# SobeyMIL/MVOC

Measured on AMD Instinct MI355X. Metric: UNet3D denoising steps/sec, 16x512^2 frames, inversion+compose, higher is better.
Workload: dtype f16

## Files before the change

### mvoc_amd/build.py

```python
import hashlib
import os
import subprocess
import sys

HERE = os.path.dirname(os.path.abspath(__file__))
CSRC = os.path.join(HERE, "csrc")
LIB = os.path.join(HERE, "libmvoc_hip.so")
SOURCES = ["runtime.hip", "gemm.hip", "gemm8.hip", "attention.hip", "tfused.hip", "xslin.hip", "norm.hip", "pnp.hip", "pnp_variants2.hip", "pnp_warp.hip", "stem.hip", "comm.hip",
           "pnp_bilinear.hip", "collage.hip"]
HIPCC = os.environ.get("HIPCC", "/opt/rocm/bin/hipcc")
LAB = os.environ.get("MVOC_BUILD_LAB") == "1"
if LAB:
    LIB = os.path.join(HERE, "libmvoc_hip_lab.so")
VARIANT = os.environ.get("MVOC_BUILD_VARIANT", "")
VARIANT_DEFS = os.environ.get("MVOC_BUILD_DEFS", "").split()
if VARIANT:
    LIB = os.path.join(HERE, f"libmvoc_hip_{VARIANT}.so")
FLAGS = ["--offload-arch=gfx950", "-O3", "-std=c++17", "-fPIC", "-fno-gpu-rdc", "-Wall", "-Wno-unused-function",
         "-ffp-contract=on", "-Rpass-analysis=kernel-resource-usage"]
EXTRA_FLAGS = {"attention.hip": ["-mllvm", "-amdgpu-mfma-vgpr-form"], "gemm.hip": ["-mllvm", "-amdgpu-mfma-vgpr-form"],
               "gemm8.hip": ["-mllvm", "-amdgpu-mfma-vgpr-form", "-falign-loops=64"], "tfused.hip": ["-mllvm", "-amdgpu-mfma-vgpr-form"],
               "xslin.hip": ["-mllvm", "-amdgpu-mfma-vgpr-form"]}


def _digest():
    h = hashlib.sha256()
    for f in sorted(x for x in os.listdir(CSRC) if x.endswith((".hip", ".h"))) + ["../../include/mvoc_hip.h"]:
        with open(os.path.join(CSRC, f), "rb") as fh:
            h.update(fh.read())
    h.update((" ".join(FLAGS + VARIANT_DEFS) + repr(sorted(EXTRA_FLAGS.items()))).encode())
    return h.hexdigest()


def build(force=False, verbose=True):
    stamp = LIB + ".stamp"
    dig = _digest()
    if not force and os.path.exists(LIB) and os.path.exists(stamp) and open(stamp).read() == dig:
        return LIB
    objs = []
    procs = []
    shared = b"".join(open(os.path.join(CSRC, f), "rb").read() for f in sorted(os.listdir(CSRC)) if f.endswith(".h"))
    shared += open(os.path.join(HERE, "..", "include", "mvoc_hip.h"), "rb").read()
    for src in SOURCES:
        obj = os.path.join(CSRC, src.replace(".hip", f".{VARIANT}.o" if VARIANT else (".lab.o" if LAB else ".o")))
        objs.append(obj)
        cmd = [HIPCC, *FLAGS, *(["-DMVOC_PP_LAB"] if LAB else []), *VARIANT_DEFS, *EXTRA_FLAGS.get(src, []), "-c", os.path.join(CSRC, src), "-o", obj]
        od = hashlib.sha256(open(os.path.join(CSRC, src), "rb").read() + shared + " ".join(cmd).encode()).hexdigest()
        ostamp = obj + ".stamp"
        if not force and os.path.exists(obj) and os.path.exists(ostamp) and open(ostamp).read() == od:
            continue
        if verbose:
            print(" ".join(cmd), flush=True)
        procs.append((src, subprocess.Popen(cmd, stdout=subprocess.PIPE, stderr=subprocess.STDOUT, text=True), ostamp, od))
    failed = False
    for src, p, ostamp, od in procs:
        out, _ = p.communicate()
        remarks = "\n".join(l for l in out.splitlines() if "-Rpass-analysis=kernel-resource-usage" in l)
        out = "\n".join(l for l in out.splitlines() if "-Rpass-analysis=kernel-resource-usage" not in l)
        with open(ostamp.replace(".stamp", ".res.txt"), "w") as fh:
            fh.write(remarks + "\n")
        if out.strip() and verbose:
            print(out)
        if p.returncode != 0:
            failed = True
            print(f"hipcc failed on {src}:\n{out}", file=sys.stderr)
        else:
            with open(ostamp, "w") as fh:
                fh.write(od)
    if failed:
        raise RuntimeError("libmvoc_hip.so: compilation failed")
    cmd = [HIPCC, "--offload-arch=gfx950", "-shared", "-fPIC", "-o", LIB, *objs, "-ldl"]
    if verbose:
        print(" ".join(cmd), flush=True)
    subprocess.run(cmd, check=True)
    with open(stamp, "w") as fh:
        fh.write(dig)
    return LIB


if __name__ == "__main__":
    build(force="--force" in sys.argv)
```

### mvoc_amd/csrc/gemm.hip

```cpp
#include <stdlib.h>

#include "gemm_args.h"

namespace {

constexpr int BK = 32;
constexpr int ROWB = 80;

struct RowInfo {
  int m;
  int y0, x0;
  int img;
};

template <int WN, int WM, int TN, int TM>
__device__ __forceinline__ void gemm_epilogue(const GemmArgs& p, f32x16 (&acc)[TN][TM], int n0, int m0, int wn, int wm,
                                              int r, int h, const float* lnstat = nullptr) {
#pragma unroll
  for (int j = 0; j < TM; ++j) {
    const int m = m0 + (wm * TM + j) * 32 + r;
    if (m >= p.M) continue;
    const half_t* ra = p.rowadd ? p.rowadd + (size_t)(m / p.rowadd_div) * p.ld_rowadd : nullptr;
    const half_t* rs = p.resid ? p.resid + (size_t)m * p.ldr : nullptr;
    half_t* orow = p.out + (size_t)m * p.ldo;
// ... 703 lines not shown
  for (int i = 0; i < 8; ++i) {
    const int m = blockIdx.x * 256 + rg + 32 * i;
    f32x4 a = {0.f, 0.f, 0.f, 0.f};
    for (int s = 0; s < p.split_k; ++s) a += *reinterpret_cast<const f32x4*>(p.ws + ((size_t)s * p.M + m) * p.N + n);
    float v[4];
#pragma unroll
    for (int e = 0; e < 4; ++e) v[e] = r16(a[e] + bs[e]);
    if (p.rowadd) {
      const half4_t ra = *reinterpret_cast<const half4_t*>(p.rowadd + (size_t)(m / p.rowadd_div) * p.ld_rowadd + n);
#pragma unroll
      for (int e = 0; e < 4; ++e) v[e] = r16(v[e] + (float)ra[e]);
    }
    if (p.resid) {
      const half4_t rs = *reinterpret_cast<const half4_t*>(p.resid + (size_t)m * p.ldr + n);
#pragma unroll
      for (int e = 0; e < 4; ++e) v[e] = r16(v[e] + (float)rs[e]);
    }
    const half4_t o4 = {(half_t)v[0], (half_t)v[1], (half_t)v[2], (half_t)v[3]};
    *reinterpret_cast<half4_t*>(p.out + (size_t)m * p.ldo + n) = o4;
#pragma unroll
    for (int e = 0; e < 4; ++e) {
      const float f = (float)o4[e];
      sx[e] += f;
      sq[e] += f * f;
    }
  }
#pragma unroll
  for (int e = 0; e < 4; ++e) {
    ls[rg][4 * cq + e] = sx[e];
    lq[rg][4 * cq + e] = sq[e];
  }
  __syncthreads();
  if (tid < 64) {
    const int c = tid & 31;
    const float(*src)[33] = tid < 32 ? ls : lq;
    float acc = 0.f;
#pragma unroll
    for (int g = 0; g < 32; ++g) acc += src[g][c];
    p.stats[((size_t)blockIdx.x * p.n_store + blockIdx.y * 32 + c) * 2 + (tid >> 5)] = acc;
  }
}

template <int WN, int WM, int TN, int TM, int NST = 2, int PF = 0, int BKK = 64, int PLAIN = 0>
int launch_glds(const GemmArgs& a0, hipStream_t s) {
  GemmArgs a = a0;
  constexpr int BN = WN * TN * 32, BM = WM * TM * 32;
  a.n_tiles = (a.N + BN - 1) / BN;
  a.m_tiles = (a.M + BM - 1) / BM;
  const long nblk = (long)a.n_tiles * a.m_tiles;
  if (nblk <= 0 || nblk > 0x7fffffffL) {
    mvoc_set_error("gemm: grid of %ld blocks", nblk);
    return -2;
  }
  constexpr bool HOT = (WN == 2 && WM == 2 && TN == 2 && TM == 2) || (WN == 1 && WM == 4 && TM == 1 && (TN == 2 || TN == 5));
  if (HOT && a.epi_lds && !a.ln_s && a.act == MVOC_ACT_NONE && a.split_k == 1) {
    if constexpr (HOT) {
      hipLaunchKernelGGL((gemm_glds_kernel<WN, WM, TN, TM, NST, PF, BKK, PLAIN, 1>), dim3((unsigned)nblk), dim3(WN * WM * 64), 0, s, a);
      return mvoc_check_launch("gemm_glds_kernel (plain epilogue)");
    }
  }
  hipLaunchKernelGGL((gemm_glds_kernel<WN, WM, TN, TM, NST, PF, BKK, PLAIN>), dim3((unsigned)(nblk * a.split_k)), dim3(WN * WM * 64), 0, s, a);
  if (a.split_k > 1) {
    if (a.stats) {
      hipLaunchKernelGGL(splitk_reduce_sums_kernel, dim3((unsigned)(a.M / 256), (unsigned)(a.N / 32)), dim3(256), 0, s, a);
    } else {
      const long nthr = (long)a.M * (a.N / 4);
      hipLaunchKernelGGL(splitk_reduce_kernel, dim3((unsigned)((nthr + 255) / 256)), dim3(256), 0, s, a);
    }
  }
  return mvoc_check_launch("gemm_glds_kernel");
}

}

extern "C" size_t mvoc_gemm_workspace_bytes(int64_t m, int64_t n, int64_t k) {
  if (m <= 0 || n <= 0 || k < 2048 || m > 8192) return 0;
  return (size_t)8 * (size_t)m * (size_t)n * sizeof(float);
}

namespace {
thread_local int g_sums_written = 0;
thread_local int g_rowmom_bx = 0;
const bool g_trace = getenv("MVOC_GEMM_TRACE") != nullptr;
}
extern "C" int mvoc_gemm_chan_sums_written(void) { return g_sums_written; }
extern "C" int mvoc_gemm_row_moments_written(void) { return g_rowmom_bx; }

namespace {
bool sums_reduce_ok(const mvoc_gemm_desc* d) {
  return d->ldo % 4 == 0 && ((uintptr_t)d->out & 7) == 0 && (!d->resid || (d->ldr % 4 == 0 && ((uintptr_t)d->resid & 7) == 0)) &&
         (!d->rowadd || (d->ld_rowadd % 4 == 0 && ((uintptr_t)d->rowadd & 7) == 0));
}

int gemm_dispatch(const mvoc_gemm_desc* d, void* stream) {
  g_sums_written = 0;
  g_rowmom_bx = 0;
  MVOC_REQUIRE(d && d->a && d->w && d->out, -1, "gemm: null operand");
  MVOC_REQUIRE(d->m > 0 && d->n > 0 && d->k > 0, -1, "gemm: empty problem m=%ld n=%ld k=%ld", (long)d->m, (long)d->n,
               (long)d->k);
  MVOC_REQUIRE(d->m < (1LL << 31) && d->n < (1 << 24) && d->k < (1 << 24), -2, "gemm: problem too large");
  MVOC_REQUIRE(d->n % 32 == 0 && d->k % BK == 0, -2, "gemm: n (%ld) must be a multiple of 32 and k (%ld) of %d",
               (long)d->n, (long)d->k, BK);
  MVOC_REQUIRE(d->cin > 0 && d->cin % 8 == 0 && d->c1 % 8 == 0 && d->c1 <= d->cin, -2,
               "gemm: cin (%d) and c1 (%d) must be multiples of 8", d->cin, d->c1);
  MVOC_REQUIRE(d->a2 || d->c1 == d->cin, -1, "gemm: c1 < cin needs a second source");
  MVOC_REQUIRE(d->a_mode >= 0 && d->a_mode <= 2, -1, "gemm: bad a_mode %d", d->a_mode);
  MVOC_REQUIRE(d->ldo % 4 == 0 && (d->resid == nullptr || d->ldr % 4 == 0), -2, "gemm: ldo/ldr must be multiples of 4");
  GemmArgs a;
  memset(&a, 0, sizeof(a));
  a.a = (const half_t*)d->a; a.a2 = (const half_t*)d->a2; a.w = (const half_t*)d->w; a.out = (half_t*)d->out;
  a.bias = (const half_t*)d->bias; a.rowadd = (const half_t*)d->rowadd; a.resid = (const half_t*)d->resid;
  a.M = (int)d->m; a.N = (int)d->n; a.K = (int)d->k;
  a.n_store = d->n_store > 0 ? d->n_store : (int)d->n;
  a.ldo = d->ldo; a.ldr = d->ldr; a.ld_rowadd = d->ld_rowadd; a.rowadd_div = d->rowadd_div > 0 ? d->rowadd_div : 1;
  a.a_mode = d->a_mode; a.lda = d->lda; a.lda2 = d->lda2; a.c1 = d->c1; a.cin = d->cin;
  a.nimg = d->nimg; a.hout = d->hout; a.wout = d->wout; a.hsrc = d->hsrc; a.wsrc = d->wsrc;
  a.stride = d->stride > 0 ? d->stride : 1; a.upsample = d->upsample;
  a.pad = d->pad_mode == 1 ? 0 : 1;
  a.hup = d->upsample ? d->hup : d->hsrc; a.wup = d->upsample ? d->wup : d->wsrc;
  a.ups_sh = d->upsample ? (float)d->hsrc / (float)d->hup : 1.f;
  a.ups_sw = d->upsample ? (float)d->wsrc / (float)d->wup : 1.f;
  a.frames = d->frames; a.hw = d->hw; a.act = d->act;
  a.split_k = 1; a.k_per_split = (int)d->k; a.ws = nullptr;
  a.ln_s = (const float*)d->ln_rowsum; a.ln_c = (const float*)d->ln_bias; a.ln_eps = d->ln_eps;
  a.ln_stats = (const float*)d->ln_stats;
  {
    const int ns = d->act == MVOC_ACT_GEGLU ? (int)d->n / 2 : (d->n_store > 0 ? d->n_store : (int)d->n);
    a.epi_lds = d->ldo % 8 == 0 && ns % 8 == 0 && ((uintptr_t)d->out & 15) == 0 &&
                (d->resid == nullptr || (d->ldr % 8 == 0 && ((uintptr_t)d->resid & 15) == 0));
  }
  if (d->a_mode == MVOC_A_CONV3X3) {
    MVOC_REQUIRE(d->nimg > 0 && d->hout > 0 && d->wout > 0 && d->hsrc > 0 && d->wsrc > 0, -1, "gemm: conv dims");
    MVOC_REQUIRE((int64_t)d->nimg * d->hout * d->wout == d->m, -1, "gemm: conv m != nimg*hout*wout");
    MVOC_REQUIRE(d->upsample == 2 || d->k >= 9 * (int64_t)d->cin, -1, "gemm: conv k < 9*cin");
    MVOC_REQUIRE(d->pad_mode == 0 || (d->pad_mode == 1 && !d->upsample), -1, "gemm: pad_mode %d", d->pad_mode);
    if (d->upsample == 2) {
      const int64_t spr = (int64_t)d->nimg * d->hsrc * d->wsrc;
      MVOC_REQUIRE(d->hup == 2 * d->hsrc && d->wup == 2 * d->wsrc && d->hout == d->hup && d->wout == d->wup && d->stride <= 1 &&
                       d->k == 4 * (int64_t)d->cin && spr % 256 == 0 && d->a2 == nullptr && d->resid == nullptr && d->rowadd == nullptr &&
                       d->act == MVOC_ACT_NONE && !d->ln_rowsum && d->split_k <= 1 && d->m >= 1024 && (d->tile == 0 || d->tile == 81),
                   -2, "gemm: upsample == 2 (sub-pixel) needs an exact 2x upsample, k == 4 cin, one source, nimg * hsrc * wsrc %% 256 == 0, "
                       "the plain epilogue, no split-K and m >= 1024");
      a.subpx = 1;
      a.sp_rows = (int)spr;
      a.hout = d->hsrc; a.wout = d->wsrc;
      a.hup = d->hsrc; a.wup = d->wsrc;
    }
  } else if (d->a_mode == MVOC_A_TEMPORAL3) {
    MVOC_REQUIRE(d->frames > 0 && d->hw > 0 && d->m % ((int64_t)d->frames * d->hw) == 0, -1, "gemm: temporal dims");
    MVOC_REQUIRE(d->k == 3 * (int64_t)d->cin, -1, "gemm: temporal k != 3*cin");
  } else {
    MVOC_REQUIRE(d->k == d->cin, -1, "gemm: plain mode needs cin == k");
  }
  if (d->act == MVOC_ACT_GEGLU) {
    MVOC_REQUIRE(d->n % 64 == 0, -2, "gemm: GEGLU needs n %% 64 == 0");
    a.n_store = (int)d->n / 2;
  }
  hipStream_t s = (hipStream_t)stream;
  const double flops = 2.0 * (double)d->m * (double)d->n * (double)d->k;
  MvocProfScope prof(MVOC_FAM_GEMM, s, flops);
  const bool glds_ok = d->k % 64 == 0 && d->cin % 64 == 0 && d->c1 % 64 == 0 &&
                       (d->a_mode != MVOC_A_CONV3X3 || d->k == (d->upsample == 2 ? 4 : 9) * (int64_t)d->cin);
  if (d->ln_rowsum) {
    MVOC_REQUIRE(d->ln_bias && d->ln_stats && glds_ok && d->a_mode == MVOC_A_PLAIN && d->a2 == nullptr && d->split_k <= 1 &&
                     (d->tile == 0 || d->tile >= 11),
                 -2, "gemm: LayerNorm folding needs the rows' statistics (ln_stats, mvoc_row_stats_f16) and the plain single-source "
                     "direct-to-LDS path (k %% 64 == 0), no split-K");
  }
  int tile = d->tile;
  int model_sk = 0, g8_sk = 0;
  const int conc = d->concurrency < 1 ? 1 : (d->concurrency > 8 ? 8 : d->concurrency);
  const int64_t rows_a = d->a_mode == MVOC_A_CONV3X3 ? (int64_t)d->nimg * d->hsrc * d->wsrc : d->m;
  const int64_t lim = (int64_t)1 << 31;
  const bool g8_ok = glds_ok && a.epi_lds && (a.n_store % 8 == 0) &&
                     rows_a * d->lda * 2 < lim && (d->a2 == nullptr || rows_a * d->lda2 * 2 < lim) &&
                     (int64_t)d->n * d->k * 2 < lim &&
                     (int64_t)d->m * d->ldo * 2 < lim && (!d->resid || (int64_t)d->m * d->ldr * 2 < lim) &&
                     ((uintptr_t)d->bias & 15) == 0 && ((uintptr_t)d->ln_rowsum & 15) == 0 && ((uintptr_t)d->ln_bias & 15) == 0 &&
                     (!d->rowadd || (((uintptr_t)d->rowadd & 15) == 0 && d->ld_rowadd % 8 == 0 && a.rowadd_div >= 64)) &&
                     (!d->upsample || (d->act == MVOC_ACT_NONE && !d->ln_rowsum));
  if (d->k_order) {
    MVOC_REQUIRE(d->k_order == 1 && d->a_mode != MVOC_A_PLAIN && !d->upsample && g8_ok && d->m >= 1024 && (tile == 0 || tile == 82) &&
                     d->k == (d->a_mode == MVOC_A_CONV3X3 ? 9 : 3) * (int64_t)d->cin && d->n % 320 == 0 && d->act == MVOC_ACT_NONE &&
                     !d->ln_rowsum && d->split_k <= 1 &&
                     (d->a_mode != MVOC_A_CONV3X3 || (a.stride == 1 && a.pad == 1 && d->hsrc == d->hout && d->wsrc == d->wout)),
                 -2, "gemm: k_order = 1 (chunk-major K) is a form of the 320-wide eight-phase tile: conv3x3 (stride 1, pad 1) / temporal3, "
                     "n %% 320 == 0, cin, c1 %% 64 == 0, no upsample, no activation, no split-K, m >= 1024, 16-byte addressable operands < 2 GB");
    a.korder = 1;
    tile = 82;
  }
  if (a.subpx) {
    MVOC_REQUIRE(g8_ok, -2, "gemm: the sub-pixel upsample conv runs on the eight-phase tiles only (k, cin %% 64 == 0, 16-byte addressable output)");
    tile = 81;
  }
  if (tile == 0 && g8_ok && d->m >= 1024 && d->k >= 256) {
    auto eff = [&](int bx, double rate) {
      const int64_t nt = (d->n + bx - 1) / bx, blocks = ((d->m + 255) / 256) * nt * conc;
      return (double)d->n / (double)(nt * bx) * (double)blocks / (double)(((blocks + 255) / 256) * 256) * rate;
    };
    const double e81 = eff(256, 1.0);
    const double e82 = (d->act != MVOC_ACT_GEGLU && d->n % 320 == 0) ? eff(320, 0.85) : 0.0;
    if (e81 >= 0.55 || e82 >= 0.55) {
      tile = e82 > e81 ? 82 : 81;
    } else if (d->workspace && d->split_k == 0 && !d->ln_rowsum && d->act != MVOC_ACT_GEGLU && d->k >= 3840) {
      const int64_t blocks = ((d->m + 255) / 256) * ((d->n + 255) / 256) * conc;
      if (blocks >= 64 && blocks < 190) {
        for (int sk = (int)(256 / blocks) > 4 ? 4 : (int)(256 / blocks); sk >= 2; --sk)
          if (d->k % (64 * sk) == 0 && (size_t)sk * d->m * d->n * 4 <= d->workspace_bytes) {
            tile = 81;
            g8_sk = sk;
            break;
          }
      }
    }
  }
  if (tile == 0 && glds_ok) {
    if (d->k <= 640 && d->m > 2048 && !(d->act == MVOC_ACT_GEGLU && d->k > 320 && d->m >= 16384)) {
      tile = (d->act == MVOC_ACT_GEGLU || d->n % 128 == 0 || d->n > 320 || d->n % 160) ? 61 : 62;
    } else if (d->act == MVOC_ACT_GEGLU) {
      tile = 11;
    } else if (d->m <= 2048 && !(d->workspace && d->k >= 2048)) {
      tile = 13;
    } else {
      static const struct { int tile, bn, bm, slots; float rate; } cand[] = {
          {12, 160, 128, 512, 950.f}, {11, 128, 128, 512, 890.f}, {64, 160, 256, 512, 1090.f}};
      const bool can_split = d->workspace && d->split_k == 0 && !d->ln_rowsum;
      double best = 0;
      for (const auto& c : cand) {
        if (d->n % c.bn) continue;
        if (c.bm == 256 && d->m < 65536) continue;
        const long blocks = ((d->m + c.bm - 1) / c.bm) * ((d->n + c.bn - 1) / c.bn) * conc;
        int sk = 1;
        if (can_split && blocks < 384 && c.bm == 128)
          while (sk < 8 && blocks * sk < 512 && d->k % (64 * sk * 2) == 0 && d->k / (sk * 2) >= 512) sk *= 2;
        if (sk > 1 && (size_t)sk * d->m * d->n * 4 > d->workspace_bytes) sk = 1;
        const double w = (double)(blocks * sk) / c.slots;
        const double full = (double)(long)w, frac = w - full;
        const double waves = full + (frac > 0 ? 0.3 + 0.7 * frac : 0.0);
        double cost = waves * c.slots * 2.0 * c.bm * c.bn * (double)(d->k / sk) / (c.rate * 1e6);
        if (sk > 1) cost += 5.0 + 2.0 * sk * (double)d->m * d->n * 4.0 / 3.0e6;
        if (tile == 0 || cost < best) { best = cost; tile = c.tile; model_sk = sk; }
      }
      if (tile == 0) tile = 13;
    }
  }
  if (tile == 0) {
    if (d->act == MVOC_ACT_GEGLU) tile = 1;
    else if (d->n % 160 == 0 && d->m >= 2048) tile = 2;
    else if (d->n % 128 == 0 && d->m >= 2048) tile = 1;
    else tile = 3;
  }
  if (tile >= 11 && d->act != MVOC_ACT_GEGLU && d->workspace && d->split_k != 1 && !d->ln_rowsum) {
    const bool t8 = tile == 81 || tile == 82;
    const int bm = t8 || tile == 64 ? 256 : 128;
    const int bn = tile == 82 ? 320 : tile == 81 ? 256 : (tile % 10 == 2 || tile == 64) ? 160 : (tile % 10 == 3 ? 64 : 128);
    const long blocks = ((d->m + bm - 1) / bm) * ((d->n + bn - 1) / bn) * conc;
    int sk = d->split_k > 1 ? d->split_k : 1;
    if (model_sk > 0) {
      sk = model_sk;
    } else if (d->split_k == 0 && blocks < 384) {
      while (sk < 8 && blocks * sk < 512 && d->k % (64 * sk * 2) == 0 && d->k / (sk * 2) >= 512) sk *= 2;
    }
    if (sk > 1 && d->k % (64 * sk) == 0 && (size_t)sk * d->m * d->n * 4 <= d->workspace_bytes) {
      a.split_k = sk;
      a.k_per_split = (int)(d->k / sk);
      a.ws = (float*)d->workspace;
      if (!t8 && d->chan_sums && d->act == MVOC_ACT_NONE && a.M % 256 == 0 && a.N % 32 == 0 && a.n_store == a.N && sums_reduce_ok(d)) {
        a.stats = (float*)d->chan_sums;
        g_sums_written = 1;
      }
    }
  }
  if (g_trace) {
    fprintf(stderr, "[mvoc gemm] mode %d m %ld n %ld k %ld cin %d act %d resid %d ln %d -> tile %d split_k %d\n", d->a_mode, (long)d->m,
            (long)d->n, (long)d->k, d->cin, d->act, d->resid != nullptr, d->ln_rowsum != nullptr, tile, (tile == 81 || tile == 82) ? (d->tile ? d->split_k : (g8_sk > 1 ? g8_sk : 1)) : a.split_k);
  }
  {
    if (tile == 81 || tile == 82) {
      MVOC_REQUIRE(g8_ok && !(tile == 82 && d->act == MVOC_ACT_GEGLU), -2,
                   "gemm: tiles 81 / 82 need k, cin, c1 %% 64 == 0, 16-byte addressable outputs, row statistics, operands < 2 GB "
                   "(82: no GEGLU)");
      a.split_k = 1; a.k_per_split = (int)d->k; a.ws = nullptr;
      if (g8_sk > 1) {
        a.split_k = g8_sk; a.k_per_split = (int)(d->k / g8_sk); a.ws = (float*)d->workspace;
      }
      if (d->tile != 0) {
        if (d->split_k > 1 && d->workspace && d->act != MVOC_ACT_GEGLU && !d->ln_rowsum && d->k % (64 * d->split_k) == 0 &&
            (size_t)d->split_k * d->m * d->n * 4 <= d->workspace_bytes) {
          a.split_k = d->split_k; a.k_per_split = (int)(d->k / d->split_k); a.ws = (float*)d->workspace;
        }
      }
      if (d->chan_sums && a.split_k == 1 && d->act == MVOC_ACT_NONE && a.M % 256 == 0 && !a.subpx) {
        a.stats = (float*)d->chan_sums;
        g_sums_written = 1;
      }
      if (d->row_moments && a.split_k == 1 && d->act != MVOC_ACT_GEGLU && a.n_store == a.N && !a.subpx) {
        MVOC_REQUIRE(d->row_moments_ld >= (a.N + 255) / 256, -2, "gemm: row_moments_ld %d < ceil(n / 256)", d->row_moments_ld);
        a.rowmom = (float*)d->row_moments;
        a.rowmom_ld = d->row_moments_ld;
      }
      int bx_used = 0;
      const int rc = mvoc_launch_gemm8(a, tile == 81 ? 256 : 320, s, &bx_used);
      if (rc == 0 && a.rowmom) g_rowmom_bx = bx_used;
      if (rc == 0 && a.split_k > 1) {
        if (d->chan_sums && d->act == MVOC_ACT_NONE && a.M % 256 == 0 && a.N % 32 == 0 && a.n_store == a.N && sums_reduce_ok(d)) {
          a.stats = (float*)d->chan_sums;
          g_sums_written = 1;
          hipLaunchKernelGGL(splitk_reduce_sums_kernel, dim3((unsigned)(a.M / 256), (unsigned)(a.N / 32)), dim3(256), 0, s, a);
          return mvoc_check_launch("splitk_reduce_sums_kernel");
        }
        const long nthr = (long)a.M * (a.N / 4);
        hipLaunchKernelGGL(splitk_reduce_kernel, dim3((unsigned)((nthr + 255) / 256)), dim3(256), 0, s, a);
        return mvoc_check_launch("splitk_reduce_kernel");
      }
      return rc;
    }
  }
  if (glds_ok && d->a_mode == MVOC_A_PLAIN && d->a2 != nullptr && !d->ln_rowsum) {
    switch (tile) {
      case 11: return launch_glds<2, 2, 2, 2, 2, 0, 64, 2>(a, s);
      case 12: if (d->act != MVOC_ACT_GEGLU) return launch_glds<1, 4, 5, 1, 2, 0, 64, 2>(a, s); break;
      case 13: return launch_glds<1, 4, 2, 1, 2, 0, 64, 2>(a, s);
      case 61: return launch_glds<2, 2, 2, 2, 2, 0, 32, 2>(a, s);
      case 62: if (d->act != MVOC_ACT_GEGLU) return launch_glds<1, 4, 5, 1, 2, 0, 32, 2>(a, s); break;
      default: break;
    }
  }
  if (glds_ok && d->a_mode == MVOC_A_PLAIN && d->a2 == nullptr && !d->upsample) {
    switch (tile) {
      case 11: return launch_glds<2, 2, 2, 2, 2, 0, 64, 1>(a, s);
      case 12: if (d->act != MVOC_ACT_GEGLU) return launch_glds<1, 4, 5, 1, 2, 0, 64, 1>(a, s); break;
      case 13: return launch_glds<1, 4, 2, 1, 2, 0, 64, 1>(a, s);
      case 61: return launch_glds<2, 2, 2, 2, 2, 0, 32, 1>(a, s);
      case 62: if (d->act != MVOC_ACT_GEGLU) return launch_glds<1, 4, 5, 1, 2, 0, 32, 1>(a, s); break;
      default: break;
    }
  }
  switch (tile) {
    case 1: return launch<2, 2, 2, 2>(a, s);
    case 2:
      MVOC_REQUIRE(d->act != MVOC_ACT_GEGLU, -2, "gemm: tile 2 cannot do GEGLU");
      return launch<1, 4, 5, 1>(a, s);
    case 3:
      if (d->act == MVOC_ACT_GEGLU) return launch<1, 4, 2, 1>(a, s);
      return launch<2, 2, 1, 2>(a, s);
    case 4: return launch<1, 4, 2, 1>(a, s);
    case 11:
      MVOC_REQUIRE(glds_ok, -2, "gemm: glds tiles need k, cin, c1 %% 64 == 0");
      return launch_glds<2, 2, 2, 2>(a, s);
    case 12:
      MVOC_REQUIRE(glds_ok && d->act != MVOC_ACT_GEGLU, -2, "gemm: tile 12 needs k, cin, c1 %% 64 == 0 and no GEGLU");
      return launch_glds<1, 4, 5, 1>(a, s);
    case 13:
      MVOC_REQUIRE(glds_ok, -2, "gemm: glds tiles need k, cin, c1 %% 64 == 0");
      return launch_glds<1, 4, 2, 1>(a, s);
    case 61:
      MVOC_REQUIRE(glds_ok, -2, "gemm: tile 61 needs k, cin, c1 %% 64 == 0");
      return launch_glds<2, 2, 2, 2, 2, 0, 32>(a, s);
    case 62:
      MVOC_REQUIRE(glds_ok && d->act != MVOC_ACT_GEGLU, -2, "gemm: tile 62 needs k, cin, c1 %% 64 == 0, no GEGLU");
      return launch_glds<1, 4, 5, 1, 2, 0, 32>(a, s);
    case 64:
      MVOC_REQUIRE(glds_ok && d->act != MVOC_ACT_GEGLU, -2, "gemm: tile 64 needs k, cin, c1 %% 64 == 0, no GEGLU");
      return launch_glds<1, 4, 5, 2, 2, 0, 32>(a, s);
    default: mvoc_set_error("gemm: unknown tile %d", tile); return -1;
  }
}
}

extern "C" int mvoc_gemm_f16(const mvoc_gemm_desc* d, void* stream) {
  const int rc = gemm_dispatch(d, stream);
  if (rc != 0) g_sums_written = g_rowmom_bx = 0;
  return rc;
}
```

### mvoc_amd/csrc/gemm_args.h

```cpp
#pragma once
#include "common.h"

struct GemmArgs {
  const half_t* a;
  const half_t* a2;
  const half_t* w;
  half_t* out;
  const half_t* bias;
  const half_t* rowadd;
  const half_t* resid;
  int M, N, K, n_store;
  int ldo, ldr, ld_rowadd, rowadd_div;
  int a_mode, lda, lda2, c1, cin;
  int nimg, hout, wout, hsrc, wsrc, stride, upsample, hup, wup;
  int pad;
  float ups_sh, ups_sw;
  int frames, hw;
  int act;
  int n_tiles, m_tiles;
  const float* ln_s;
  const float* ln_c;
  const float* ln_stats;
  float ln_eps;
  int split_k, k_per_split;
  float* ws;
  unsigned mg_nt, mg_sk, mg_hwout, mg_wout, mg_hw, mg_fr, mg_ra, mg_band;
  int sh_nt, sh_sk, sh_hwout, sh_wout, sh_hw, sh_fr, sh_ra, sh_band;
  int band;
  int tmap_t, sh_tm;
  unsigned mg_tm;
  float* stats;
  float* rowmom;
  int rowmom_ld;
  int subpx, sp_rows;
  int korder;
  int epi_lds;
};


int mvoc_launch_gemm8(const GemmArgs& a, int bx, hipStream_t s, int* bx_used = nullptr);
```

Measured before the change: 25.58.

## Add persistent 256-wide eight-phase GEMM kernel and auto-select it for multi-wave linears

Adds a new persistent GEMM kernel (gemm8p) that launches one block per compute unit and loops over output tiles. It prefetches the next tile's operands while running the current tile's epilogue, to hide per-tile prologue and epilogue latency and tail effects. The dispatcher selects it automatically for plain linears with K up to 1280 when the tile count exceeds the CU count, and it can be forced with tile 83 or disabled with an environment variable. The cost is a large amount of new hand-scheduled kernel code, and results or performance may differ from the existing gemm8 path.

```diff
diff --git a/mvoc_amd/build.py b/mvoc_amd/build.py
--- a/mvoc_amd/build.py
+++ b/mvoc_amd/build.py
@@ -7,6 +7,7 @@
 CSRC = os.path.join(HERE, "csrc")
 LIB = os.path.join(HERE, "libmvoc_hip.so")
 SOURCES = ["runtime.hip", "gemm.hip", "gemm8.hip", "attention.hip", "tfused.hip", "xslin.hip", "norm.hip", "pnp.hip", "pnp_variants2.hip", "pnp_warp.hip", "stem.hip", "comm.hip",
+           "gemm8p.hip",
            "pnp_bilinear.hip", "collage.hip"]
 HIPCC = os.environ.get("HIPCC", "/opt/rocm/bin/hipcc")
 LAB = os.environ.get("MVOC_BUILD_LAB") == "1"
@@ -20,7 +21,8 @@
          "-ffp-contract=on", "-Rpass-analysis=kernel-resource-usage"]
 EXTRA_FLAGS = {"attention.hip": ["-mllvm", "-amdgpu-mfma-vgpr-form"], "gemm.hip": ["-mllvm", "-amdgpu-mfma-vgpr-form"],
                "gemm8.hip": ["-mllvm", "-amdgpu-mfma-vgpr-form", "-falign-loops=64"], "tfused.hip": ["-mllvm", "-amdgpu-mfma-vgpr-form"],
-               "xslin.hip": ["-mllvm", "-amdgpu-mfma-vgpr-form"]}
+               "xslin.hip": ["-mllvm", "-amdgpu-mfma-vgpr-form"],
+               "gemm8p.hip": ["-mllvm", "-amdgpu-mfma-vgpr-form", "-falign-loops=64"]}
 
 
 def _digest():
diff --git a/mvoc_amd/csrc/gemm.hip b/mvoc_amd/csrc/gemm.hip
--- a/mvoc_amd/csrc/gemm.hip
+++ b/mvoc_amd/csrc/gemm.hip
@@ -809,6 +809,15 @@
 thread_local int g_sums_written = 0;
 thread_local int g_rowmom_bx = 0;
 const bool g_trace = getenv("MVOC_GEMM_TRACE") != nullptr;
+const bool g_g8p_auto = !(getenv("MVOC_G8P") && atoi(getenv("MVOC_G8P")) == 0);
+int g8p_cus() {
+  static const int n = [] {
+    int dev = 0, v = 0;
+    if (hipGetDevice(&dev) != hipSuccess || hipDeviceGetAttribute(&v, hipDeviceAttributeMultiprocessorCount, dev) != hipSuccess) v = 0;
+    return v;
+  }();
+  return n;
+}
 }
 extern "C" int mvoc_gemm_chan_sums_written(void) { return g_sums_written; }
 extern "C" int mvoc_gemm_row_moments_written(void) { return g_rowmom_bx; }
@@ -856,6 +865,10 @@
     a.epi_lds = d->ldo % 8 == 0 && ns % 8 == 0 && ((uintptr_t)d->out & 15) == 0 &&
                 (d->resid == nullptr || (d->ldr % 8 == 0 && ((uintptr_t)d->resid & 15) == 0));
   }
+  if (d->tile == 83) {
+    const char* why = d->split_k > 1 ? "no split-K" : d->k_order ? "no upsample and no chunk-major K" : mvoc_gemm8p_scope(a);
+    MVOC_REQUIRE(!why, -2, "gemm: tile 83 (gemm8p, the persistent 256-wide eight-phase form) needs %s", why);
+  }
   if (d->a_mode == MVOC_A_CONV3X3) {
     MVOC_REQUIRE(d->nimg > 0 && d->hout > 0 && d->wout > 0 && d->hsrc > 0 && d->wsrc > 0, -1, "gemm: conv dims");
     MVOC_REQUIRE((int64_t)d->nimg * d->hout * d->wout == d->m, -1, "gemm: conv m != nimg*hout*wout");
@@ -894,7 +907,8 @@
                  -2, "gemm: LayerNorm folding needs the rows' statistics (ln_stats, mvoc_row_stats_f16) and the plain single-source "
                      "direct-to-LDS path (k %% 64 == 0), no split-K");
   }
-  int tile = d->tile;
+  const bool forced83 = d->tile == 83;
+  int tile = forced83 ? 81 : d->tile;
   int model_sk = 0, g8_sk = 0;
   const int conc = d->concurrency < 1 ? 1 : (d->concurrency > 8 ? 8 : d->concurrency);
   const int64_t rows_a = d->a_mode == MVOC_A_CONV3X3 ? (int64_t)d->nimg * d->hsrc * d->wsrc : d->m;
@@ -1025,6 +1039,17 @@
         MVOC_REQUIRE(d->row_moments_ld >= (a.N + 255) / 256, -2, "gemm: row_moments_ld %d < ceil(n / 256)", d->row_moments_ld);
         a.rowmom = (float*)d->row_moments;
         a.rowmom_ld = d->row_moments_ld;
+      }
+      constexpr int G8P_MAX_K = 1280;
+      bool pers = forced83;
+      if (!pers && d->tile == 0 && tile == 81 && g_g8p_auto && g8_sk <= 1 && d->k <= G8P_MAX_K && g8p_cus() > 0 && !mvoc_gemm8p_scope(a))
+        pers = (int64_t)((a.M + 255) / 256) * ((a.N + 255) / 256) > g8p_cus();
+      if (pers) {
+        MVOC_REQUIRE(g8p_cus() > 0, -3, "gemm: tile 83 (gemm8p) could not query the device's compute units");
+        if (g_trace) fprintf(stderr, "[mvoc gemm]   -> gemm8p, the persistent form, on %d blocks\n", g8p_cus());
+        const int rc = mvoc_launch_gemm8p(a, g8p_cus(), s);
+        if (rc == 0 && a.rowmom) g_rowmom_bx = 256;
+        return rc;
       }
       int bx_used = 0;
       const int rc = mvoc_launch_gemm8(a, tile == 81 ? 256 : 320, s, &bx_used);
diff --git a/mvoc_amd/csrc/gemm8p.hip b/mvoc_amd/csrc/gemm8p.hip
--- /dev/null
+++ b/mvoc_amd/csrc/gemm8p.hip
@@ -0,0 +1,522 @@
+#include <stdlib.h>
+
+#include <type_traits>
+
+#include "gemm_args.h"
+
+namespace {
+
+typedef __fp16 fp16x4_t __attribute__((__vector_size__(4 * sizeof(__fp16))));
+
+constexpr unsigned GP_OOB = 0x80000000u;
+__device__ const uint4 gp_zero16 = {0u, 0u, 0u, 0u};
+
+#define GP_BAR()                         \
+  do {                                   \
+    __builtin_amdgcn_sched_barrier(0);   \
+    __builtin_amdgcn_s_barrier();        \
+    __builtin_amdgcn_sched_barrier(0);   \
+  } while (0)
+
+__device__ __forceinline__ unsigned gp_udiv(unsigned n, unsigned mg, int sh) { return sh < 0 ? n : __umulhi(n, mg) >> sh; }
+
+template <int N>
+__device__ __forceinline__ void gp_wait_vm() {
+  asm volatile("s_waitcnt vmcnt(%0)" ::"n"(N) : "memory");
+}
+
+template <int EPI>
+__global__ __launch_bounds__(512) void gemm8p_kernel(const GemmArgs p) {
+  constexpr int XT = 4;
+  constexpr int XQ = XT * 16, XH = 2 * XQ, BX = 4 * XQ;
+  constexpr int XB = XH * 128, YB = 128 * 128;
+  constexpr int KB = 2 * XB + YB;
+  constexpr int OX0 = 0, OY1 = XB, OX1 = XB + YB;
+  constexpr int B0 = 0, YS0 = KB, T_B = KB + YB, B1 = T_B + 8192, YS1 = B1 + KB;
+  constexpr int SMEM = 163840;
+  constexpr int PITCH = XQ * 2 + 16;
+  constexpr int RA_ROWS = 5;
+  constexpr int NB = BX / 8, NL = BX / 4, TOT = NB + 2 * NL + RA_ROWS * NB;
+  constexpr int T_LS = T_B + NB * 16, T_LC = T_LS + NL * 16, T_RA = T_LC + NL * 16;
+  constexpr int EPI0 = B1;
+  constexpr int S_OFF = EPI0 + 8 * 64 * PITCH;
+  constexpr int R_OFF = S_OFF + 4 * BX * 8;
+  static_assert(TOT <= 512 && TOT * 16 <= 8192, "epilogue table");
+  static_assert(YS1 + YB <= S_OFF && R_OFF + 4 * 256 * 8 == SMEM, "LDS layout");
+  __shared__ __attribute__((aligned(1024))) char smem[SMEM];
+#define GP_KB(P) ((P) ? B1 : B0)
+#define GP_YS(P) ((P) ? YS1 : YS0)
+
+  const int tid = threadIdx.x;
+  const int lane = tid & 63;
+  const int wave = __builtin_amdgcn_readfirstlane(tid >> 6);
+  const int wr = wave >> 2, wc = wave & 3;
+  const unsigned ntot = (unsigned)p.n_tiles * (unsigned)p.m_tiles;
+  const int nk = p.K / 64;
+
+  auto coords = [&](unsigned v, unsigned& mtile, unsigned& ntile) {
+    const unsigned logical = xcd_remap(v, ntot);
+    if (p.band > 1) {
+      const unsigned per = (unsigned)p.band * (unsigned)p.n_tiles;
+      const unsigned b_ = gp_udiv(logical, p.mg_band, p.sh_band);
+      const unsigned idx = logical - b_ * per;
+      const unsigned rows = min((unsigned)p.band, (unsigned)p.m_tiles - b_ * (unsigned)p.band);
+      ntile = idx / rows;
+      mtile = b_ * (unsigned)p.band + (idx - ntile * rows);
+    } else {
+      mtile = gp_udiv(logical, p.mg_nt, p.sh_nt);
+      ntile = logical - mtile * (unsigned)p.n_tiles;
+    }
+  };
+
+  auto fresh_tid = [&]() {
+    int l = tid;
+    asm volatile("" : "+v"(l));
+    return l;
+  };
+  auto fresh_lane = [&]() { return fresh_tid() & 63; };
+  const __amdgpu_buffer_rsrc_t rs_w = __builtin_amdgcn_make_buffer_rsrc((void*)p.w, 0, (int)((size_t)p.N * p.K * 2), 0x00020000);
+  const __amdgpu_buffer_rsrc_t rs_y = __builtin_amdgcn_make_buffer_rsrc((void*)p.a, 0, (int)((size_t)p.M * p.lda * 2), 0x00020000);
+  unsigned xoff[2], yoff;
+  const unsigned xh1 = (unsigned)XQ * (unsigned)p.K * 2u;
+  const unsigned yrow32 = 32u * (unsigned)p.lda * 2u;
+  int xso0 = 0, xso1 = 0, yso = 0;
+  const int wbase = wave * 1024;
+  auto set_offsets = [&](int m0_, int n0_) {
+    const int ln = fresh_lane();
+    const int lrow = ln >> 3, pos = ln & 7;
+    const int cch = (pos ^ ((4 * wave + (lrow >> 1)) & 7)) * 8;
+    int lda2 = p.lda * 2;
+    asm volatile("" : "+s"(lda2));
+#pragma unroll
+    for (int q = 0; q < 2; ++q) {
+      const int lr = 8 * (wave + 8 * q) + lrow;
+      const int row = n0_ + (lr / XQ) * (2 * XQ) + (lr % XQ);
+      xoff[q] = (unsigned)(((size_t)row * p.K + cch) * 2);
+    }
+    const int lr0 = 8 * wave + lrow;
+    yoff = (unsigned)__umul24((unsigned)(m0_ + (lr0 >> 5) * 64 + (lr0 & 31)), (unsigned)lda2) + (unsigned)(cch * 2);
+  };
+  auto opaque_add = [&](unsigned v, unsigned sc) -> unsigned {
+    unsigned r;
+    asm volatile("v_add_u32 %0, %1, %2" : "=v"(r) : "s"(sc), "v"(v));
+    return r;
+  };
+#define GP_LDS(off) ((__attribute__((address_space(3))) void*)(smem + (off)))
+#define GP_ISSUE_X(h, base, so)                                                                                          \
+  do {                                                                                                                   \
+    _Pragma("unroll") for (int q = 0; q < 2; ++q)                                                                        \
+        __builtin_amdgcn_raw_ptr_buffer_load_lds(rs_w, GP_LDS((base) + wbase + q * 8192), 16, (int)((h) ? opaque_add(xoff[q], xh1) : xoff[q]), so, 0, 0); \
+    so += 128;                                                                                                           \
+  } while (0)
+#define GP_ISSUE_Y(h, base)                                                                                              \
+  do {                                                                                                                   \
+    _Pragma("unroll") for (int q = 0; q < 2; ++q)                                                                        \
+        __builtin_amdgcn_raw_ptr_buffer_load_lds(rs_y, GP_LDS((base) + wbase + q * 8192), 16, (int)((h) + q ? opaque_add(yoff, ((h) + 4 * q) * yrow32) : yoff), yso, 0, 0); \
+  } while (0)
+#define GP_ISSUE_TILE0()                                                         \
+  do {                                                                           \
+    xso0 = xso1 = yso = 0;                                                       \
+    GP_ISSUE_X(0, B0 + OX0, xso0); GP_ISSUE_X(1, B0 + OX1, xso1);                \
+    GP_ISSUE_Y(0, YS0); GP_ISSUE_Y(1, B0 + OY1);                                 \
+    yso += 128;                                                                  \
+  } while (0)
+
+  unsigned vtile = blockIdx.x, mtile, ntile;
+  coords(vtile, mtile, ntile);
+  int n0 = (int)ntile * BX, m0 = (int)mtile * 256;
+  set_offsets(m0, n0);
+  GP_ISSUE_TILE0();
+  __builtin_amdgcn_sched_barrier(0);
+
+  const char *xr0, *xr1, *yr0, *yr1;
+  auto set_fragment_pointers = [&]() {
+    const int ln = fresh_lane();
+    const int fr = ln & 15, fg = ln >> 4;
+    const int sw = fr >> 1;
+    xr0 = smem + (wr * XQ + fr) * 128 + (fg ^ sw) * 16;
+    xr1 = smem + (wr * XQ + fr) * 128 + ((4 + fg) ^ sw) * 16;
+    yr0 = smem + (wc * 32 + fr) * 128 + (fg ^ sw) * 16;
+    yr1 = smem + (wc * 32 + fr) * 128 + ((4 + fg) ^ sw) * 16;
+  };
+#define GP_LDP(ptr, off) (*reinterpret_cast<const half8_t*>((ptr) + (off)))
+  half8_t xf[XT][2], yf0[2][2], yf1[2][2];
+  f32x4 acc[2][2][XT][2];
+#define GP_RDX(off)                                             \
+  _Pragma("unroll") for (int i = 0; i < XT; ++i) {              \
+    xf[i][0] = GP_LDP(xr0, (off) + i * 2048);                   \
+    xf[i][1] = GP_LDP(xr1, (off) + i * 2048);                   \
+  }
+#define GP_RDY(dst, off)                                        \
+  _Pragma("unroll") for (int j = 0; j < 2; ++j) {               \
+    dst[j][0] = GP_LDP(yr0, (off) + j * 2048);                  \
+    dst[j][1] = GP_LDP(yr1, (off) + j * 2048);                  \
+  }
+#define GP_MMA(A, B, YF)                                                                                              \
+  do {                                                                                                                \
+    __builtin_amdgcn_s_setprio(1);                                                                                    \
+    _Pragma("unroll") for (int s = 0; s < 2; ++s) _Pragma("unroll") for (int i = 0; i < XT; ++i)                     \
+        _Pragma("unroll") for (int j = 0; j < 2; ++j)                                                                 \
+            acc[A][B][i][j] = __builtin_amdgcn_mfma_f32_16x16x32_f16(xf[i][s], YF[j][s], acc[A][B][i][j], 0, 0, 0);   \
+    __builtin_amdgcn_s_setprio(0);                                                                                    \
+  } while (0)
+
+#define GP_KTILE(P, t)                                                                                 \
+  do {                                                                                                 \
+    GP_RDY(yf0, GP_YS(P));                                                                             \
+    asm volatile("" ::: "memory");                                                                     \
+    __builtin_amdgcn_sched_barrier(0);                                                                 \
+    GP_RDX(GP_KB(P) + OX0);                                                                            \
+    asm volatile("" ::: "memory");                                                                     \
+    __builtin_amdgcn_sched_barrier(0);                                                                 \
+    if ((t) + 1 < nk) GP_ISSUE_X(1, GP_KB(1 - (P)) + OX1, xso1);                                       \
+    __builtin_amdgcn_sched_barrier(0);                                                                 \
+    asm volatile("s_waitcnt lgkmcnt(%0)" ::"n"(2 * XT) : "memory");                                    \
+    GP_BAR();                                                                                          \
+    GP_MMA(0, 0, yf0);                                                                                 \
+    GP_BAR();                                                                                          \
+    GP_RDY(yf1, GP_KB(P) + OY1);                                                                       \
+    asm volatile("" ::: "memory");                                                                     \
+    __builtin_amdgcn_sched_barrier(0);                                                                 \
+    if ((t) + 2 < nk) GP_ISSUE_Y(0, GP_YS(P));                                                         \
+    GP_BAR();                                                                                          \
+    GP_MMA(0, 1, yf1);                                                                                 \
+    GP_BAR();                                                                                          \
+    GP_RDX(GP_KB(P) + OX1);                                                                            \
+    asm volatile("" ::: "memory");                                                                     \
+    __builtin_amdgcn_sched_barrier(0);                                                                 \
+    if ((t) + 2 < nk) GP_ISSUE_X(0, GP_KB(P) + OX0, xso0);                                             \
+    GP_BAR();                                                                                          \
+    GP_MMA(1, 1, yf1);                                                                                 \
+    GP_BAR();                                                                                          \
+    if ((t) + 2 < nk) {                                                                                \
+      GP_ISSUE_Y(1, GP_KB(P) + OY1);                                                                   \
+      yso += 128;                                                                                      \
+      gp_wait_vm<6>();                                                                     \
+    } else if ((t) + 2 == nk) {                                                                        \
+      gp_wait_vm<0>();                                                                                 \
+    }                                                                                                  \
+    GP_BAR();                                                                                          \
+    GP_MMA(1, 0, yf0);                                                                                 \
+    GP_BAR();                                                                                          \
+  } while (0)
+
+  constexpr bool GG = EPI == 3, LNF = EPI != 1, RADD = EPI == 1;
+  constexpr bool geglu = EPI == 3;
+  constexpr int nchunk = geglu ? 4 : XT * 2;
+  char* epi = smem + EPI0 + wave * (64 * PITCH);
+  typedef unsigned u32x4 __attribute__((ext_vector_type(4)));
+  const __amdgpu_buffer_rsrc_t rs_o = __builtin_amdgcn_make_buffer_rsrc((void*)p.out, 0, (int)((size_t)p.M * p.ldo * 2), 0x00020000);
+  const __amdgpu_buffer_rsrc_t rs_r =
+      __builtin_amdgcn_make_buffer_rsrc((void*)(p.resid ? p.resid : p.out), 0, p.resid ? (int)((size_t)p.M * p.ldr * 2) : 0, 0x00020000);
+
+  bool first = true;
+  for (;;) {
+    set_offsets(m0, n0);
+    set_fragment_pointers();
+    GP_ISSUE_Y(0, YS1); GP_ISSUE_X(0, B1 + OX0, xso0); GP_ISSUE_Y(1, B1 + OY1);
+    yso += 128;
+    if (first) gp_wait_vm<6>();
+    else gp_wait_vm<6 + 2 * nchunk>();
+    __builtin_amdgcn_sched_barrier(0);
+    const unsigned ra_row0 = RADD && p.rowadd ? gp_udiv((unsigned)m0, p.mg_ra, p.sh_ra) : 0u;
+    {
+      const int tid = fresh_tid();
+      unsigned long long a_ls = (unsigned long long)p.ln_s, a_lc = (unsigned long long)p.ln_c;
+      asm volatile("" : "+s"(a_ls), "+s"(a_lc));
+      const void* src = &gp_zero16;
+      if (tid < NB) {
+        const int n = n0 + tid * 8;
+        if (!LNF && p.bias && n < p.N) src = p.bias + n;
+      } else if (tid < NB + 2 * NL) {
+        const int c = tid - NB, v = c >= NL;
+        const int n = n0 + (c - v * NL) * 4;
+        if (LNF && n < p.N) src = reinterpret_cast<const float*>(v ? a_lc : a_ls) + n;
+      } else if (tid < TOT) {
+        const int c = tid - NB - 2 * NL;
+        const int r = c / NB, n = n0 + (c - r * NB) * 8;
+        const unsigned ra_rows = RADD && p.rowadd ? gp_udiv((unsigned)min(m0 + 255, p.M - 1), p.mg_ra, p.sh_ra) - ra_row0 + 1u : 0u;
+        if (RADD && (unsigned)r < ra_rows && n < p.n_store) src = p.rowadd + (size_t)(ra_row0 + r) * p.ld_rowadd + n;
+      }
+      if (wave * 64 < TOT)
+        __builtin_amdgcn_global_load_lds((const __attribute__((address_space(1))) void*)src, GP_LDS(T_B + wbase), 16, 0, 0);
+    }
+    float2 ln_st[2][2];
+    if constexpr (LNF) {
+      const int fr_ = fresh_lane() & 15;
+#pragma unroll
+      for (int b = 0; b < 2; ++b)
+#pragma unroll
+        for (int j = 0; j < 2; ++j) {
+          const int m = m0 + wc * 64 + b * 32 + j * 16 + fr_;
+          const float* src = p.ln_stats + 2 * (size_t)(m < p.M ? m : p.M - 1);
+          asm volatile("global_load_dwordx2 %0, %1, off" : "=v"(ln_st[b][j]) : "v"(src) : "memory");
+        }
+    }
+    GP_BAR();
+    if (wr == 1) GP_BAR();
+#pragma unroll
+    for (int a = 0; a < 2; ++a)
+#pragma unroll
+      for (int b = 0; b < 2; ++b)
+#pragma unroll
+        for (int i = 0; i < XT; ++i)
+#pragma unroll
+          for (int j = 0; j < 2; ++j)
+#pragma unroll
+            for (int e = 0; e < 4; ++e) {
+              float z;
+              asm volatile("v_mov_b32 %0, 0" : "=v"(z));
+              acc[a][b][i][j][e] = z;
+            }
+
+    int t = 0;
+#pragma unroll 1
+    for (; t + 1 < nk; t += 2) {
+      GP_KTILE(0, t);
+      GP_KTILE(1, t + 1);
+    }
+    if (t < nk) GP_KTILE(0, t);
+    if (wr == 0) GP_BAR();
+
+    const int lane_e = fresh_lane();
+    const int fr = lane_e & 15, g = lane_e >> 4;
+    float ln_mu[2][2], ln_rs[2][2];
+    int raoff[2][2];
+#pragma unroll
+    for (int b = 0; b < 2; ++b)
+#pragma unroll
+      for (int j = 0; j < 2; ++j) {
+        const int m = m0 + wc * 64 + b * 32 + j * 16 + fr;
+        const int ms = m < p.M ? m : p.M - 1;
+        ln_mu[b][j] = 0.f; ln_rs[b][j] = 1.f;
+        if constexpr (LNF) {
+          asm volatile("" : "+v"(ln_st[b][j]));
+          ln_mu[b][j] = ln_st[b][j].x; ln_rs[b][j] = ln_st[b][j].y;
+        }
+        raoff[b][j] = RADD && p.rowadd ? (int)(gp_udiv((unsigned)ms, p.mg_ra, p.sh_ra) - ra_row0) * (BX * 2) : 0;
+      }
+    auto nq_of = [&](int a) { return n0 + wr * XH + a * XQ; };
+    auto chunk_off = [&](int a, int ln, int it, int ld) -> unsigned {
+      const int nbase = geglu ? nq_of(a) / 2 : nq_of(a);
+      const int idx = ln + 64 * it;
+      const int px = idx / nchunk, c = idx - px * nchunk;
+      const int m = m0 + wc * 64 + px;
+      const int n = nbase + c * 8;
+      const bool ok = n < p.n_store;
+      return ok ? (unsigned)(m * ld + n) * 2u : GP_OOB;
+    };
+    u32x4 r0[nchunk], r1[nchunk];
+#pragma unroll
+    for (int it = 0; it < nchunk; ++it) r0[it] = __builtin_amdgcn_raw_buffer_load_b128(rs_r, chunk_off(0, lane_e, it, p.ldr), 0, 0);
+#pragma unroll
+    for (int it = 0; it < nchunk; ++it) r1[it] = __builtin_amdgcn_raw_buffer_load_b128(rs_r, chunk_off(1, lane_e, it, p.ldr), 0, 0);
+    __builtin_amdgcn_sched_barrier(0);
+    vtile += gridDim.x;
+    const bool has_next = vtile < ntot;
+    int m0n = 0, n0n = 0;
+    unsigned ntile_n = 0;
+    if (has_next) {
+      unsigned mt;
+      coords(vtile, mt, ntile_n);
+      n0n = (int)ntile_n * BX; m0n = (int)mt * 256;
+      set_offsets(m0n, n0n);
+      GP_ISSUE_TILE0();
+    }
+    __builtin_amdgcn_sched_barrier(0);
+
+    auto arith = [&](auto A_) {
+      constexpr int a = decltype(A_)::value;
+      const int cb = wr * XH + a * XQ + 4 * g;
+      if constexpr (GG) {
+#pragma unroll
+        for (int i = 0; i < 2; ++i) {
+          const int c = cb + i * 16;
+          const f32x4 sh = *reinterpret_cast<const f32x4*>(smem + T_LS + c * 4), sg = *reinterpret_cast<const f32x4*>(smem + T_LS + (c + 32) * 4);
+          const f32x4 ch = *reinterpret_cast<const f32x4*>(smem + T_LC + c * 4), cg = *reinterpret_cast<const f32x4*>(smem + T_LC + (c + 32) * 4);
+#pragma unroll
+          for (int b = 0; b < 2; ++b)
+#pragma unroll
+            for (int j = 0; j < 2; ++j) {
+              half4_t o;
+#pragma unroll
+              for (int e = 0; e < 4; ++e) {
+                const float av = acc[a][b][i][j][e], ag = acc[a][b][i + 2][j][e];
+                const float hv = r16(ln_rs[b][j] * (av - ln_mu[b][j] * sh[e]) + ch[e]);
+                const float gv = r16(ln_rs[b][j] * (ag - ln_mu[b][j] * sg[e]) + cg[e]);
+                o[e] = (half_t)(hv * r16(gelu_fast_f(gv)));
+              }
+              *reinterpret_cast<half4_t*>(epi + (b * 32 + j * 16 + fr) * PITCH + (i * 16 + 4 * g) * 2) = o;
+            }
+        }
+      } else {
+#pragma unroll
+        for (int i = 0; i < XT; ++i) {
+          const int c = cb + i * 16;
+          const half4_t b4 = *reinterpret_cast<const half4_t*>(smem + T_B + c * 2);
+          f32x4 s4 = {0.f, 0.f, 0.f, 0.f}, c4 = s4;
+          if constexpr (LNF) { s4 = *reinterpret_cast<const f32x4*>(smem + T_LS + c * 4); c4 = *reinterpret_cast<const f32x4*>(smem + T_LC + c * 4); }
+#pragma unroll
+          for (int b = 0; b < 2; ++b)
+#pragma unroll
+            for (int j = 0; j < 2; ++j) {
+              float x[4];
+#pragma unroll
+              for (int e = 0; e < 4; ++e)
+                x[e] = r16(LNF ? ln_rs[b][j] * (acc[a][b][i][j][e] - ln_mu[b][j] * s4[e]) + c4[e] : acc[a][b][i][j][e] + (float)b4[e]);
+              if constexpr (RADD) {
+                const half4_t t4 = *reinterpret_cast<const half4_t*>(smem + T_RA + raoff[b][j] + c * 2);
+#pragma unroll
+                for (int e = 0; e < 4; ++e) x[e] = r16(x[e] + (float)t4[e]);
+              }
+              half4_t o;
+#pragma unroll
+              for (int e = 0; e < 4; ++e) o[e] = (half_t)x[e];
+              *reinterpret_cast<half4_t*>(epi + (b * 32 + j * 16 + fr) * PITCH + (i * 16 + 4 * g) * 2) = o;
+            }
+        }
+      }
+      asm volatile("s_waitcnt lgkmcnt(0)" ::: "memory");
+    };
+    auto readback_store = [&](int a, const u32x4 (&rr)[nchunk]) {
+      const int lane2 = fresh_lane();
+#pragma unroll
+      for (int it = 0; it < nchunk; ++it) {
+        const int idx = lane2 + 64 * it;
+        const int px = idx / nchunk, c = idx - px * nchunk;
+        half8_t v = *reinterpret_cast<const half8_t*>(epi + px * PITCH + c * 16);
+        const half8_t r8 = __builtin_bit_cast(half8_t, rr[it]);
+        if (p.resid) {
+#pragma unroll
+          for (int e = 0; e < 8; ++e) v[e] = (half_t)((float)v[e] + (float)r8[e]);
+        }
+        __builtin_amdgcn_raw_buffer_store_b128(__builtin_bit_cast(u32x4, v), rs_o, chunk_off(a, lane2, it, p.ldo), 0, 2);
+        if (p.stats || p.rowmom) *reinterpret_cast<half8_t*>(epi + px * PITCH + c * 16) = v;
+      }
+      asm volatile("s_waitcnt lgkmcnt(0)" ::: "memory");
+    };
+    auto stats_pass = [&](int a) {
+      const half8_t ones = {(half_t)1.f, (half_t)1.f, (half_t)1.f, (half_t)1.f, (half_t)1.f, (half_t)1.f, (half_t)1.f, (half_t)1.f};
+      const int kg = lane_e >> 4, n = lane_e & 15;
+      float* so = reinterpret_cast<float*>(smem + S_OFF) + (wc * BX + wr * XH + a * XQ) * 2;
+#pragma unroll
+      for (int cb = 0; cb < XT; ++cb) {
+        f32x4 dg = {0.f, 0.f, 0.f, 0.f}, dsum = dg;
+#pragma unroll
+        for (int ps = 0; ps < 2; ++ps) {
+          const char* va = epi + (32 * ps + 8 * kg + (n >> 2)) * PITCH + (cb * 16 + 4 * (n & 3)) * 2;
+          const fp16x4_t lo = __builtin_amdgcn_ds_read_tr16_b64_v4f16((__attribute__((address_space(3))) fp16x4_t*)va);
+          const fp16x4_t hi = __builtin_amdgcn_ds_read_tr16_b64_v4f16((__attribute__((address_space(3))) fp16x4_t*)(va + 4 * PITCH));
+          half8_t f;
+#pragma unroll
+          for (int e = 0; e < 4; ++e) { f[e] = (half_t)lo[e]; f[4 + e] = (half_t)hi[e]; }
+          dg = __builtin_amdgcn_mfma_f32_16x16x32_f16(f, f, dg, 0, 0, 0);
+          dsum = __builtin_amdgcn_mfma_f32_16x16x32_f16(ones, f, dsum, 0, 0, 0);
+        }
+        const float sq = (n & 3) == 0 ? dg[0] : (n & 3) == 1 ? dg[1] : (n & 3) == 2 ? dg[2] : dg[3];
+        if (kg == (n >> 2)) *reinterpret_cast<float2*>(so + (cb * 16 + n) * 2) = float2{dsum[0], sq};
+      }
+    };
+    auto rowmom_pass = [&](int a) {
+      const half8_t ones = {(half_t)1.f, (half_t)1.f, (half_t)1.f, (half_t)1.f, (half_t)1.f, (half_t)1.f, (half_t)1.f, (half_t)1.f};
+      const int kg = lane_e >> 4, n = lane_e & 15;
+      float* ro = reinterpret_cast<float*>(smem + R_OFF) + ((wr * 2 + a) * 256 + wc * 64) * 2;
+#pragma unroll
+      for (int rb = 0; rb < 4; ++rb) {
+        f32x4 dg = {0.f, 0.f, 0.f, 0.f}, dsum = dg;
+#pragma unroll
+        for (int ks = 0; ks * 32 < XQ; ++ks) {
+          const half8_t f = *reinterpret_cast<const half8_t*>(epi + (rb * 16 + n) * PITCH + (ks * 32 + kg * 8) * 2);
+          dg = __builtin_amdgcn_mfma_f32_16x16x32_f16(f, f, dg, 0, 0, 0);
+          dsum = __builtin_amdgcn_mfma_f32_16x16x32_f16(ones, f, dsum, 0, 0, 0);
+        }
+        const float sq = (n & 3) == 0 ? dg[0] : (n & 3) == 1 ? dg[1] : (n & 3) == 2 ? dg[2] : dg[3];
+        if (kg == (n >> 2)) *reinterpret_cast<float2*>(ro + (rb * 16 + n) * 2) = float2{dsum[0], sq};
+      }
+    };
+    {
+      using I0 = std::integral_constant<int, 0>;
+      using I1 = std::integral_constant<int, 1>;
+      arith(I0{});
+      __builtin_amdgcn_sched_barrier(0);
+      readback_store(0, r0);
+      __builtin_amdgcn_sched_barrier(0);
+      if (p.stats) stats_pass(0);
+      if (p.rowmom) rowmom_pass(0);
+      __builtin_amdgcn_sched_barrier(0);
+      arith(I1{});
+      __builtin_amdgcn_sched_barrier(0);
+      readback_store(1, r1);
+      if (p.stats) stats_pass(1);
+      if (p.rowmom) rowmom_pass(1);
+      asm volatile("s_waitcnt lgkmcnt(0)" ::: "memory");
+      GP_BAR();
+      const int i = fresh_tid();
+      if (p.stats) {
+        if (n0 + (i >> 1) < p.n_store) {
+          const float* si = reinterpret_cast<const float*>(smem + S_OFF) + i;
+          p.stats[((size_t)(m0 >> 8) * p.n_store + n0) * 2 + i] = ((si[0] + si[BX * 2]) + si[2 * BX * 2]) + si[3 * BX * 2];
+        }
+      }
+      if (p.rowmom) {
+        const int row = m0 + (i >> 1);
+        if (row < p.M) {
+          const float* ri = reinterpret_cast<const float*>(smem + R_OFF) + i;
+          p.rowmom[((size_t)row * p.rowmom_ld + ntile) * 2 + (i & 1)] = ((ri[0] + ri[512]) + ri[1024]) + ri[1536];
+        }
+      }
+    }
+    if (!has_next) break;
+    m0 = m0n; n0 = n0n; ntile = ntile_n;
+    first = false;
+  }
+}
+
+void gp_magic(unsigned d, unsigned& mg, int& sh) {
+  if (d <= 1) { mg = 0; sh = -1; return; }
+  int l = 0;
+  while ((1ull << l) < d) ++l;
+  mg = (unsigned)(((1ull << (31 + l)) + d - 1) / d);
+  sh = l - 1;
+}
+
+}
+
+const char* mvoc_gemm8p_scope(const GemmArgs& a) {
+  if (a.a_mode != MVOC_A_PLAIN || a.a2 || a.c1 != a.cin) return "a plain single-source linear";
+  if (a.upsample || a.subpx || a.korder) return "no upsample and no chunk-major K";
+  if (a.split_k != 1) return "no split-K";
+  if (a.K < 128 || a.K % 64) return "k a multiple of 64, at least 128";
+  const bool e1 = a.act == MVOC_ACT_NONE && !a.ln_s, e2 = a.act == MVOC_ACT_NONE && a.ln_s && !a.rowadd, e3 = a.act == MVOC_ACT_GEGLU && a.ln_s;
+  if (!e1 && !e2 && !e3) return "the bias / row-add / residual, LayerNorm-fold or LayerNorm-fold + GEGLU epilogue";
+  return nullptr;
+}
+
+int mvoc_launch_gemm8p(const GemmArgs& a0, int blocks, hipStream_t s) {
+  if (const char* why = mvoc_gemm8p_scope(a0)) {
+    mvoc_set_error("gemm8p: the persistent form needs %s", why);
+    return -2;
+  }
+  GemmArgs a = a0;
+  a.n_tiles = (a.N + 255) / 256;
+  a.m_tiles = (a.M + 255) / 256;
+  gp_magic((unsigned)a.n_tiles, a.mg_nt, a.sh_nt);
+  {
+    static const int force = getenv("MVOC_G8_BAND") ? atoi(getenv("MVOC_G8_BAND")) : 0;
+    a.band = force ? force : (a.n_tiles >= 8 ? 4 : a.n_tiles >= 4 ? 2 : 1);
+    if (a.band > a.m_tiles) a.band = 1;
+    gp_magic((unsigned)(a.band * a.n_tiles), a.mg_band, a.sh_band);
+  }
+  gp_magic((unsigned)a.rowadd_div, a.mg_ra, a.sh_ra);
+  const long ntot = (long)a.n_tiles * a.m_tiles;
+  if (ntot <= 0 || ntot > 0x7fffffffL || blocks <= 0) {
+    mvoc_set_error("gemm8p: %ld tiles on %d blocks", ntot, blocks);
+    return -2;
+  }
+  const unsigned grid = (unsigned)(ntot < blocks ? ntot : blocks);
+  const int epi = a.act == MVOC_ACT_GEGLU ? 3 : a.ln_s ? 2 : 1;
+  if (epi == 1) hipLaunchKernelGGL((gemm8p_kernel<1>), dim3(grid), dim3(512), 0, s, a);
+  else if (epi == 2) hipLaunchKernelGGL((gemm8p_kernel<2>), dim3(grid), dim3(512), 0, s, a);
+  else hipLaunchKernelGGL((gemm8p_kernel<3>), dim3(grid), dim3(512), 0, s, a);
+  return mvoc_check_launch("gemm8p_kernel");
+}
diff --git a/mvoc_amd/csrc/gemm_args.h b/mvoc_amd/csrc/gemm_args.h
--- a/mvoc_amd/csrc/gemm_args.h
+++ b/mvoc_amd/csrc/gemm_args.h
@@ -39,3 +39,6 @@
 
 
 int mvoc_launch_gemm8(const GemmArgs& a, int bx, hipStream_t s, int* bx_used = nullptr);
+
+const char* mvoc_gemm8p_scope(const GemmArgs& a);
+int mvoc_launch_gemm8p(const GemmArgs& a, int blocks, hipStream_t s);
```

New measurement: 25.68 (median of 6 runs). Within noise of the previous version (+0.4%).
